# LambdaLabsML/distributed-training-guide

Measured on AMD Instinct MI355X. Metric: tokens/sec/GPU for Llama-style causal LM at 1/2/4/8 MI355X; peak HBM per GPU, higher is better.
Workload: dtype bf16; 1 GPU; model=llama-3-8b, global_batch=24, seq_len=1024, parallelism=single

## Files before the change

distributed_training_guide_amd/_hip/attention_bwd.hip:

```cpp
#include "attention_common.h"
#include "launchers.h"

template <int D>
__global__ void __launch_bounds__(256) attn_delta_kernel(
    const short* __restrict__ dout, const short* __restrict__ o,
    float* __restrict__ delta, int B, int S, int Hq) {
  const int grp = threadIdx.x >> 4;
  const int gl = threadIdx.x & 15;
  int64_t nrows = (int64_t)B * S * Hq;
  for (int64_t row = (int64_t)blockIdx.x * 16 + grp; row < nrows;
       row += (int64_t)gridDim.x * 16) {
    const short* dp = dout + row * D;
    const short* op = o + row * D;
    float s = 0.f;
#pragma unroll
    for (int i = gl * 8; i < D; i += 16 * 8) {
      bf16x8 dv = *reinterpret_cast<const bf16x8*>(dp + i);
      bf16x8 ov = *reinterpret_cast<const bf16x8*>(op + i);
#pragma unroll
      for (int j = 0; j < 8; ++j) s += bf2f(dv[j]) * bf2f(ov[j]);
    }
#pragma unroll
    for (int off = 1; off < 16; off <<= 1) s += __shfl_xor(s, off, WAVE);
    if (gl == 0) {
      int h = (int)(row % Hq);
      int64_t bs = row / Hq;
      int sp = (int)(bs % S);
      int b = (int)(bs / S);
      delta[((int64_t)b * Hq + h) * S + sp] = s;
    }
  }
}

template <int D, bool DOC>
__global__ void __launch_bounds__(256, 2) attn_dkdv_kernel(
    const short* __restrict__ dout, const short* __restrict__ q,
    const short* __restrict__ k, const short* __restrict__ v,
    const float* __restrict__ lse, const float* __restrict__ delta,
    short* __restrict__ dk, short* __restrict__ dv, int B, int S, int Hq,
    int Hkv, float scale, const int* __restrict__ doc_end) {
  static_assert(D == 64 || D == 128, "head dim must be 64 or 128");
  __shared__ short q_lds[2][64 * D];
  __shared__ short do_lds[2][64 * D];
  __shared__ __attribute__((aligned(16))) float lse_lds[2][64];
  __shared__ __attribute__((aligned(16))) float del_lds[2][64];

  const int nkt = (S + 63) / 64;
  const int group = Hq / Hkv;

  const GroupBlock gb = xcd_remap(blockIdx.x, B * Hkv, nkt);
  const int b = gb.gid / Hkv;
  const int hkv = gb.gid % Hkv;
  const int kt = gb.within;

  const int tid = threadIdx.x;
  const int wid = tid >> 6;
  const int lane = tid & (WAVE - 1);
  const int l15 = lane & 15;
  const int lg = lane >> 4;

  const int kv0 = kt * 64 + wid * 16;
  constexpr int nd16 = D >> 4, nkc = D >> 5;
  const float c2 = scale * LOG2E;
  const int64_t strideS_q = (int64_t)Hq * D;
  const int64_t strideS_kv = (int64_t)Hkv * D;
  const short* kb = k + ((int64_t)b * S * Hkv + hkv) * D;
  const short* vb = v + ((int64_t)b * S * Hkv + hkv) * D;

  bf16x8 kf[nkc], vf[nkc];
  {
    int key = kv0 + l15;
    int keyc = key < S ? key : S - 1;
    const short* kp = kb + (int64_t)keyc * strideS_kv + lg * 8;
    const short* vp = vb + (int64_t)keyc * strideS_kv + lg * 8;
#pragma unroll
    for (int c = 0; c < nkc; ++c) {
      kf[c] = *reinterpret_cast<const bf16x8*>(kp + c * 32);
      vf[c] = *reinterpret_cast<const bf16x8*>(vp + c * 32);
    }
  }

  f32x4 dkacc[nd16], dvacc[nd16];
#pragma unroll
  for (int i = 0; i < nd16; ++i) {
    dkacc[i] = {0.f, 0.f, 0.f, 0.f};
    dvacc[i] = {0.f, 0.f, 0.f, 0.f};
  }

  const int qstart = kt * 64;
  int dend = S, dend_min = S, qcap = S;
  if (DOC) {
    const int* deb = doc_end + (int64_t)b * S;
    dend = deb[min(kv0 + l15, S - 1)];
    dend_min = deb[min(kv0, S - 1)];
    qcap = min(max(deb[min(qstart + 63, S - 1)], qstart + 1), S);
  }
  const int nqt = (qcap - qstart + 63) / 64;
  const int niter = group * nqt;

  auto stage_qdo = [&](int it, int buf) {
    const int64_t hoff = ((int64_t)b * S * Hq + hkv * group + it / nqt) * D;
    stage_tile_pair<D>(q + hoff, dout + hoff, strideS_q,
                       qstart + (it % nqt) * 64, S, q_lds[buf], do_lds[buf],
                       wid, lane);
  };
  auto stage_lse = [&](int it, int buf) {
    const int hh = hkv * group + it / nqt;
    const int qt = qstart + (it % nqt) * 64;
    if (tid < 64) {
      const float* lseb = lse + ((int64_t)b * Hq + hh) * S;
      int rr = qt + tid < S ? qt + tid : S - 1;
      lse_lds[buf][tid] = lseb[rr] * LOG2E;
    } else if (tid < 128) {
      const float* delb = delta + ((int64_t)b * Hq + hh) * S;
      int rr = qt + tid - 64 < S ? qt + tid - 64 : S - 1;
      del_lds[buf][tid - 64] = delb[rr] * scale;
    }
  };

  stage_qdo(0, 0);
  stage_lse(0, 0);
  __syncthreads();

  for (int it = 0; it < niter; ++it) {
    const int buf = it & 1;
    if (it + 1 < niter) {
      stage_qdo(it + 1, buf ^ 1);
      stage_lse(it + 1, buf ^ 1);
    }

    const int qt = qstart + (it % nqt) * 64;
    const short* ql = q_lds[buf];
    const short* dol = do_lds[buf];

    const int key = kv0 + l15;
    const bool diag = (qt < kt * 64 + 64) || (qt + 63 >= S) ||
                      (DOC && qt + 63 >= dend_min);
    u32x4 pk_p[2], pk_ds[2];
    __builtin_amdgcn_s_setprio(1);
#pragma unroll
    for (int mth = 0; mth < 2; ++mth) {
      const int qra = perm16(2 * mth, l15), qrb = perm16(2 * mth + 1, l15);
      f32x4 sa0 = {0.f, 0.f, 0.f, 0.f}, da0 = {0.f, 0.f, 0.f, 0.f};
      f32x4 sa1 = {0.f, 0.f, 0.f, 0.f}, da1 = {0.f, 0.f, 0.f, 0.f};
#pragma unroll
      for (int c = 0; c < nkc; ++c) {
        bf16x8 qa0 = *reinterpret_cast<const bf16x8*>(
            ql + st_idx(qra, c * 32 + lg * 8));
        bf16x8 qa1 = *reinterpret_cast<const bf16x8*>(
            ql + st_idx(qrb, c * 32 + lg * 8));
        bf16x8 do0 = *reinterpret_cast<const bf16x8*>(
            dol + st_idx(qra, c * 32 + lg * 8));
        bf16x8 do1 = *reinterpret_cast<const bf16x8*>(
            dol + st_idx(qrb, c * 32 + lg * 8));
        sa0 = mfma16(qa0, kf[c], sa0);
        sa1 = mfma16(qa1, kf[c], sa1);
        da0 = mfma16(do0, vf[c], da0);
        da1 = mfma16(do1, vf[c], da1);
      }
#pragma unroll
      for (int half = 0; half < 2; ++half) {
        const int mt = 2 * mth + half;
        const f32x4 sa = half ? sa1 : sa0;
        const f32x4 da = half ? da1 : da0;
        const int qoff = cpos16(mt, lg);
        const f32x4 lse4 =
            *reinterpret_cast<const f32x4*>(&lse_lds[buf][qoff]);
        const f32x4 del4 =
            *reinterpret_cast<const f32x4*>(&del_lds[buf][qoff]);
        float e[4], p[4], ds[4];
#pragma unroll
        for (int r = 0; r < 4; ++r)
          e[r] = __builtin_fmaf(sa[r], c2, -lse4[r]);
        if (diag) {
#pragma unroll
          for (int r = 0; r < 4; ++r) {
            const int qrow = qt + qoff + r;
            if (key > qrow || qrow >= S || key >= S || (DOC && qrow >= dend))
              e[r] = -INFINITY;
          }
        }
#pragma unroll
        for (int r = 0; r < 4; ++r) {
          p[r] = __builtin_amdgcn_exp2f(e[r]);
          ds[r] = p[r] * __builtin_fmaf(da[r], scale, -del4[r]);
        }
        const int kc = mt >> 1, rp = (mt & 1) * 2;
        pk_p[kc][rp + 0] = cvt_pk_bf16(p[0], p[1]);
        pk_p[kc][rp + 1] = cvt_pk_bf16(p[2], p[3]);
        pk_ds[kc][rp + 0] = cvt_pk_bf16(ds[0], ds[1]);
        pk_ds[kc][rp + 1] = cvt_pk_bf16(ds[2], ds[3]);
      }
    }

#pragma unroll
    for (int dt = 0; dt < nd16; ++dt) {
#pragma unroll
      for (int kc = 0; kc < 2; ++kc) {
        bf16x8 dofr = tr16_frag_st(dol, kc * 32 + lg * 8, dt * 16, l15);
        bf16x8 qfr = tr16_frag_st(ql, kc * 32 + lg * 8, dt * 16, l15);
        dvacc[dt] = mfma16(__builtin_bit_cast(bf16x8, pk_p[kc]), dofr,
                           dvacc[dt]);
        dkacc[dt] = mfma16(__builtin_bit_cast(bf16x8, pk_ds[kc]), qfr,
                           dkacc[dt]);
      }
    }
    __builtin_amdgcn_s_setprio(0);
    __syncthreads();
  }

#pragma unroll
  for (int r = 0; r < 4; ++r) {
    int keyw = kv0 + lg * 4 + r;
    if (keyw >= S) continue;
    short* dkp = dk + ((int64_t)b * S * Hkv + (int64_t)keyw * Hkv + hkv) * D;
    short* dvp = dv + ((int64_t)b * S * Hkv + (int64_t)keyw * Hkv + hkv) * D;
#pragma unroll
    for (int dt = 0; dt < nd16; ++dt) {
      dkp[dt * 16 + l15] = f2bf(dkacc[dt][r]);
      dvp[dt * 16 + l15] = f2bf(dvacc[dt][r]);
    }
  }
}

template <int D, bool DOC>
__global__ void __launch_bounds__(256, 2) attn_dq_kernel(
    const short* __restrict__ dout, const short* __restrict__ q,
    const short* __restrict__ k, const short* __restrict__ v,
    const float* __restrict__ lse, const float* __restrict__ delta,
    short* __restrict__ dq, int B, int S, int Hq, int Hkv, float scale,
    const int* __restrict__ doc_start) {
  static_assert(D == 64 || D == 128, "head dim must be 64 or 128");
  __shared__ short k_lds[2][KVBLK * D];
  __shared__ short v_lds[2][KVBLK * D];

  const int ntq = (S + QBLK - 1) / QBLK;
  const int gqa = Hq / Hkv;
  const int bpg = gqa * ntq;

  const GroupBlock gb = xcd_remap(blockIdx.x, B * Hkv, bpg);
  const int b = gb.gid / Hkv;
  const int hkv = gb.gid % Hkv;
  const int h = hkv * gqa + gb.within / ntq;
  const int qtile = gb.within % ntq;

  const int tid = threadIdx.x;
  const int wid = tid >> 6;
  const int lane = tid & (WAVE - 1);
  const int l15 = lane & 15;
  const int lg = lane >> 4;

  const int q0 = qtile * QBLK;
  const int rowb[2] = {qgroup_row(q0, wid, 0), qgroup_row(q0, wid, 1)};
  constexpr int nd16 = D >> 4, nkc = D >> 5;
  const float c2 = scale * LOG2E;
  const int64_t strideS_q = (int64_t)Hq * D;
  const int64_t strideS_kv = (int64_t)Hkv * D;
  const short* qb = q + ((int64_t)b * S * Hq + h) * D;
  const short* dob = dout + ((int64_t)b * S * Hq + h) * D;
  const short* kb = k + ((int64_t)b * S * Hkv + hkv) * D;
  const short* vb = v + ((int64_t)b * S * Hkv + hkv) * D;
  const float* lseb = lse + ((int64_t)b * Hq + h) * S;
  const float* delb = delta + ((int64_t)b * Hq + h) * S;

  bf16x8 qf[2][nkc], dof[2][nkc];
  float lse_r[2], del_r[2];
#pragma unroll
  for (int nq = 0; nq < 2; ++nq) {
    int qrow = rowb[nq] + l15;
    int qrc = qrow < S ? qrow : S - 1;
    const short* qp = qb + (int64_t)qrc * strideS_q + lg * 8;
    const short* dop = dob + (int64_t)qrc * strideS_q + lg * 8;
#pragma unroll
    for (int c = 0; c < nkc; ++c) {
      qf[nq][c] = *reinterpret_cast<const bf16x8*>(qp + c * 32);
      dof[nq][c] = *reinterpret_cast<const bf16x8*>(dop + c * 32);
    }
    lse_r[nq] = lseb[qrc] * LOG2E;
    del_r[nq] = delb[qrc] * scale;
  }

  f32x4 dqacc[nd16][2];
#pragma unroll
  for (int dt = 0; dt < nd16; ++dt)
#pragma unroll
    for (int nq = 0; nq < 2; ++nq) dqacc[dt][nq] = {0.f, 0.f, 0.f, 0.f};

  const int kv_end = min(S, q0 + QBLK);
  const int ntiles = (kv_end + KVBLK - 1) / KVBLK;
  int dstart[2], dsmax[2];
  const int t0 =
      doc_window<DOC>(doc_start, b, S, q0, wid, l15, dstart, dsmax);

  auto stage_kv = [&](int t, int buf) {
    stage_tile_pair<D>(kb, vb, strideS_kv, t * KVBLK, S, k_lds[buf],
                       v_lds[buf], wid, lane);
  };
  stage_kv(t0, 0);
  __syncthreads();

  for (int t = t0; t < ntiles; ++t) {
    const int kv0 = t * KVBLK;
    const int buf = tile_buf(t, t0);
    if (t + 1 < ntiles) stage_kv(t + 1, buf ^ 1);

    {
      const bool smask = (kv_end < kv0 + KVBLK);
      u32x4 pk_ds[2][2];
      const short* kl = k_lds[buf];
      const short* vl = v_lds[buf];
      __builtin_amdgcn_s_setprio(1);
#pragma unroll
      for (int mt = 0; mt < 4; ++mt) {
        const int kr = perm16(mt, l15);
        f32x4 s0 = {0.f, 0.f, 0.f, 0.f}, s1 = {0.f, 0.f, 0.f, 0.f};
        f32x4 d0 = {0.f, 0.f, 0.f, 0.f}, d1 = {0.f, 0.f, 0.f, 0.f};
#pragma unroll
        for (int c = 0; c < nkc; ++c) {
          bf16x8 ka = *reinterpret_cast<const bf16x8*>(
              kl + st_idx(kr, c * 32 + lg * 8));
          bf16x8 va = *reinterpret_cast<const bf16x8*>(
              vl + st_idx(kr, c * 32 + lg * 8));
          s0 = mfma16(ka, qf[0][c], s0);
          d0 = mfma16(va, dof[0][c], d0);
          s1 = mfma16(ka, qf[1][c], s1);
          d1 = mfma16(va, dof[1][c], d1);
        }
        const int koff = cpos16(mt, lg);
        const int kc = mt >> 1, rp = (mt & 1) * 2;
#pragma unroll
        for (int nq = 0; nq < 2; ++nq) {
          const int qrow = rowb[nq] + l15;
          const bool diag = (kv0 + KVBLK - 1 > rowb[nq]) || smask ||
                            (DOC && dsmax[nq] > kv0);
          const f32x4 sv = nq ? s1 : s0;
          const f32x4 dv = nq ? d1 : d0;
          float e[4], ds[4];
#pragma unroll
          for (int r = 0; r < 4; ++r)
            e[r] = __builtin_fmaf(sv[r], c2, -lse_r[nq]);
          if (diag) {
#pragma unroll
            for (int r = 0; r < 4; ++r) {
              const int keyr = kv0 + koff + r;
              if (keyr > qrow || keyr >= S || qrow >= S ||
                  (DOC && keyr < dstart[nq]))
                e[r] = -INFINITY;
            }
          }
#pragma unroll
          for (int r = 0; r < 4; ++r)
            ds[r] = __builtin_amdgcn_exp2f(e[r]) *
                    __builtin_fmaf(dv[r], scale, -del_r[nq]);
          pk_ds[nq][kc][rp + 0] = cvt_pk_bf16(ds[0], ds[1]);
          pk_ds[nq][kc][rp + 1] = cvt_pk_bf16(ds[2], ds[3]);
        }
      }

#pragma unroll
      for (int dt = 0; dt < nd16; ++dt) {
#pragma unroll
        for (int kc = 0; kc < 2; ++kc) {
          bf16x8 kfr = tr16_frag_st(kl, kc * 32 + lg * 8, dt * 16, l15);
          dqacc[dt][0] = mfma16(__builtin_bit_cast(bf16x8, pk_ds[0][kc]),
                                kfr, dqacc[dt][0]);
          dqacc[dt][1] = mfma16(__builtin_bit_cast(bf16x8, pk_ds[1][kc]),
                                kfr, dqacc[dt][1]);
        }
      }
      __builtin_amdgcn_s_setprio(0);
    }
    __syncthreads();
  }

#pragma unroll
  for (int nq = 0; nq < 2; ++nq) {
#pragma unroll
    for (int r = 0; r < 4; ++r) {
      int qrow = rowb[nq] + lg * 4 + r;
      if (qrow >= S) continue;
      short* dqp = dq + ((int64_t)b * S * Hq + (int64_t)qrow * Hq + h) * D;
#pragma unroll
      for (int dt = 0; dt < nd16; ++dt) {
        dqp[dt * 16 + l15] = f2bf(dqacc[dt][nq][r]);
      }
    }
  }
}

namespace {
template <int D, bool DOC>
void bwd_launch(const short* dout, const short* q, const short* k,
                const short* v, const short* o, const float* lse,
                float* delta, short* dq, short* dk, short* dv,
                const int* doc_start, const int* doc_end, int B, int S,
                int Hq, int Hkv, float scale, hipStream_t stream) {
  int64_t nrows = (int64_t)B * S * Hq;
  int64_t dwant = (nrows + 15) / 16;
  int dgrid = (int)(dwant < 2048 ? (dwant < 1 ? 1 : dwant) : 2048);
  hipLaunchKernelGGL(attn_delta_kernel<D>, dim3(dgrid), dim3(256), 0, stream,
                     dout, o, delta, B, S, Hq);
  int nkt = (S + 63) / 64;
  hipLaunchKernelGGL((attn_dkdv_kernel<D, DOC>),
                     dim3((uint32_t)((int64_t)B * Hkv * nkt)), dim3(256), 0,
                     stream, dout, q, k, v, lse, delta, dk, dv, B, S, Hq, Hkv,
                     scale, doc_end);
  int ntq = (S + QBLK - 1) / QBLK;
  hipLaunchKernelGGL((attn_dq_kernel<D, DOC>),
                     dim3((uint32_t)((int64_t)B * Hq * ntq)), dim3(256), 0,
                     stream, dout, q, k, v, lse, delta, dq, B, S, Hq, Hkv,
                     scale, doc_start);
}
}

extern "C" void attn_bwd_launch(const void* dout, const void* q, const void* k,
                                const void* v, const void* o, const float* lse,
                                float* delta, void* dq, void* dk, void* dv,
                                const int* doc_start, const int* doc_end,
                                int B, int S, int Hq, int Hkv, int D,
                                float scale, hipStream_t stream) {
  const bool doc = doc_start != nullptr;
  auto fn = doc ? (D == 64 ? bwd_launch<64, true> : bwd_launch<128, true>)
                : (D == 64 ? bwd_launch<64, false> : bwd_launch<128, false>);
  fn((const short*)dout, (const short*)q, (const short*)k, (const short*)v,
     (const short*)o, lse, delta, (short*)dq, (short*)dk, (short*)dv,
     doc_start, doc_end, B, S, Hq, Hkv, scale, stream);
}
```

distributed_training_guide_amd/_hip/attention_common.h:

```cpp
#pragma once
#include "common.h"

using bf16x8 = s16x8;

constexpr int QBLK = 128;
constexpr int KVBLK = 64;
#define LOG2E 1.4426950408889634f

__device__ __forceinline__ f32x4 mfma16(bf16x8 a, bf16x8 b, f32x4 c) {
  return __builtin_amdgcn_mfma_f32_16x16x32_bf16(a, b, c, 0, 0, 0);
}

template <int D>
__device__ __forceinline__ void stage_tile_pair(
    const short* ga, const short* gb, int64_t stride, int row0, int S,
    short* la, short* lb, int wid, int lane) {
  constexpr int ncw = D >> 5;
#pragma unroll
  for (int i = 0; i < ncw; ++i) {
    const int ch = wid * ncw + i;
    int row = row0 + (ch & 1) * 32 + (lane >> 1);
    if (row >= S) row = S - 1;
    const int64_t goff =
        (int64_t)row * stride + (ch >> 1) * 16 + (lane & 1) * 8;
    __builtin_amdgcn_global_load_lds(
        (const __attribute__((address_space(1))) unsigned int*)(ga + goff),
        (LDS_AS unsigned int*)(la + ch * 512), 16, 0, 0);
    __builtin_amdgcn_global_load_lds(
        (const __attribute__((address_space(1))) unsigned int*)(gb + goff),
        (LDS_AS unsigned int*)(lb + ch * 512), 16, 0, 0);
  }
}

struct GroupBlock {
  int gid;
  int within;
};
__device__ __forceinline__ GroupBlock xcd_remap(int bid, int ngroups,
                                                int bpg) {
  if ((ngroups & 7) == 0)
    return {(bid >> 3) / bpg * 8 + (bid & 7), (bid >> 3) % bpg};
  return {bid / bpg, bid % bpg};
}

__device__ __forceinline__ int qgroup_row(int q0, int wid, int nq) {
  return q0 + nq * 64 + wid * 16;
}

template <bool DOC>
__device__ __forceinline__ int doc_window(const int* doc_start, int b, int S,
                                          int q0, int wid, int l15,
                                          int (&dstart)[2], int (&dsmax)[2]) {
  dstart[0] = dstart[1] = dsmax[0] = dsmax[1] = 0;
  if (!DOC) return 0;
  const int* dsb = doc_start + (int64_t)b * S;
#pragma unroll
  for (int nq = 0; nq < 2; ++nq) {
    dstart[nq] = dsb[min(qgroup_row(q0, wid, nq) + l15, S - 1)];
    dsmax[nq] = dsb[min(qgroup_row(q0, wid, nq) + 15, S - 1)];
  }
  return min(max(dsb[q0], 0), q0) / KVBLK;
}

__device__ __forceinline__ int tile_buf(int t, int t0) { return (t - t0) & 1; }
```

distributed_training_guide_amd/_hip/attention_fwd.hip:

```cpp
#include "attention_common.h"
#include "launchers.h"

template <int D, bool DOC>
__global__ void __launch_bounds__(256, 2) attn_fwd_kernel(
    const short* __restrict__ q, const short* __restrict__ k,
    const short* __restrict__ v, short* __restrict__ o,
    float* __restrict__ lse_out, int B, int S, int Hq, int Hkv, float scale,
    const int* __restrict__ doc_start) {
  static_assert(D == 64 || D == 128, "head dim must be 64 or 128");
  __shared__ short k_lds[2][KVBLK * D];
  __shared__ short v_lds[2][KVBLK * D];

  const int ntq = (S + QBLK - 1) / QBLK;
  const int gqa = Hq / Hkv;
  const int bpg = gqa * ntq;

  const GroupBlock gb = xcd_remap(blockIdx.x, B * Hkv, bpg);
  const int b = gb.gid / Hkv;
  const int hkv = gb.gid % Hkv;
  const int h = hkv * gqa + gb.within / ntq;
  const int qtile = gb.within % ntq;

  const int tid = threadIdx.x;
  const int wid = tid >> 6;
  const int lane = tid & (WAVE - 1);
  const int l15 = lane & 15;
  const int lg = lane >> 4;

  const int q0 = qtile * QBLK;
  const int rowb[2] = {qgroup_row(q0, wid, 0), qgroup_row(q0, wid, 1)};
  constexpr int nd16 = D >> 4;
  constexpr int nkc = D >> 5;
  const int64_t strideS_q = (int64_t)Hq * D;
  const int64_t strideS_kv = (int64_t)Hkv * D;
  const short* qb = q + ((int64_t)b * S * Hq + h) * D;
  const short* kb = k + ((int64_t)b * S * Hkv + hkv) * D;
  const short* vb = v + ((int64_t)b * S * Hkv + hkv) * D;

  bf16x8 qf[2][nkc];
#pragma unroll
  for (int nq = 0; nq < 2; ++nq) {
    int qrow = rowb[nq] + l15;
    if (qrow >= S) qrow = S - 1;
    const short* qp = qb + (int64_t)qrow * strideS_q + lg * 8;
#pragma unroll
    for (int kc = 0; kc < nkc; ++kc)
      qf[nq][kc] = *reinterpret_cast<const bf16x8*>(qp + kc * 32);
  }

  int kperm[4], ckey[4];
#pragma unroll
  for (int mt = 0; mt < 4; ++mt) {
    kperm[mt] = perm16(mt, l15);
    ckey[mt] = cpos16(mt, lg);
  }

  f32x4 oacc[nd16][2];
#pragma unroll
  for (int dt = 0; dt < nd16; ++dt)
#pragma unroll
    for (int nq = 0; nq < 2; ++nq) oacc[dt][nq] = {0.f, 0.f, 0.f, 0.f};
  float mrow[2] = {-INFINITY, -INFINITY};
  float mcrow[2] = {-INFINITY, -INFINITY};
  float lrow[2] = {0.f, 0.f};

  const int kv_end = min(S, q0 + QBLK);
  const int ntiles = (kv_end + KVBLK - 1) / KVBLK;
  const float c = scale * LOG2E;
  int dstart[2], dsmax[2];
  const int t0 =
      doc_window<DOC>(doc_start, b, S, q0, wid, l15, dstart, dsmax);

  auto stage_kv = [&](int t, int buf) {
    stage_tile_pair<D>(kb, vb, strideS_kv, t * KVBLK, S, k_lds[buf],
                       v_lds[buf], wid, lane);
  };
  stage_kv(t0, 0);
  __syncthreads();

  for (int t = t0; t < ntiles; ++t) {
    const int kv0 = t * KVBLK;
    const int buf = tile_buf(t, t0);
    if (t + 1 < ntiles) stage_kv(t + 1, buf ^ 1);


    const short* kl = k_lds[buf];
    f32x4 sfrag[4][2];
    __builtin_amdgcn_s_setprio(1);
#pragma unroll
    for (int mth = 0; mth < 2; ++mth) {
      const int kra = kperm[2 * mth], krb = kperm[2 * mth + 1];
      f32x4 a0 = {0.f, 0.f, 0.f, 0.f}, a1 = {0.f, 0.f, 0.f, 0.f};
      f32x4 b0 = {0.f, 0.f, 0.f, 0.f}, b1 = {0.f, 0.f, 0.f, 0.f};
#pragma unroll
      for (int kc = 0; kc < nkc; ++kc) {
        bf16x8 kfa = *reinterpret_cast<const bf16x8*>(
            kl + st_idx(kra, kc * 32 + lg * 8));
        bf16x8 kfb = *reinterpret_cast<const bf16x8*>(
            kl + st_idx(krb, kc * 32 + lg * 8));
        a0 = mfma16(kfa, qf[0][kc], a0);
        b0 = mfma16(kfb, qf[0][kc], b0);
        a1 = mfma16(kfa, qf[1][kc], a1);
        b1 = mfma16(kfb, qf[1][kc], b1);
      }
      sfrag[2 * mth][0] = a0;
      sfrag[2 * mth][1] = a1;
      sfrag[2 * mth + 1][0] = b0;
      sfrag[2 * mth + 1][1] = b1;
    }
    __builtin_amdgcn_s_setprio(0);

    u32x4 pk[2][2];
    float alpha[2];
#pragma unroll
    for (int nq = 0; nq < 2; ++nq) {
      const int qrow = rowb[nq] + l15;
      const bool need_mask = (kv0 + KVBLK - 1) > rowb[nq] ||
                             kv_end < kv0 + KVBLK ||
                             (DOC && dsmax[nq] > kv0);
      if (need_mask) {
#pragma unroll
        for (int mt = 0; mt < 4; ++mt)
#pragma unroll
          for (int r = 0; r < 4; ++r) {
            int key = kv0 + ckey[mt] + r;
            if (key > qrow || key >= S || (DOC && key < dstart[nq]))
              sfrag[mt][nq][r] = -INFINITY;
          }
      }
      float tmax = -INFINITY;
#pragma unroll
      for (int mt = 0; mt < 4; ++mt) {
        f32x4 s = sfrag[mt][nq];
        tmax = fmaxf(tmax, fmaxf(fmaxf(s[0], s[1]), fmaxf(s[2], s[3])));
      }
      tmax = fmaxf(tmax, __shfl_xor(tmax, 16, WAVE));
      tmax = fmaxf(tmax, __shfl_xor(tmax, 32, WAVE));
      const float mnew = fmaxf(mrow[nq], tmax);
      const float mcn = mnew * c;
      const float mc = (mnew == -INFINITY) ? 0.0f : mcn;
      alpha[nq] = __builtin_amdgcn_exp2f(mcrow[nq] - mc);
      mrow[nq] = mnew;
      mcrow[nq] = mcn;
      float psum = 0.f;
#pragma unroll
      for (int mt = 0; mt < 4; ++mt) {
        f32x4 s = sfrag[mt][nq];
        f32x4 p;
#pragma unroll
        for (int r = 0; r < 4; ++r) {
          p[r] = __builtin_amdgcn_exp2f(__builtin_fmaf(s[r], c, -mc));
          psum += p[r];
        }
        pk[nq][mt >> 1][(mt & 1) * 2 + 0] = cvt_pk_bf16(p[0], p[1]);
        pk[nq][mt >> 1][(mt & 1) * 2 + 1] = cvt_pk_bf16(p[2], p[3]);
      }
      psum += __shfl_xor(psum, 16, WAVE);
      psum += __shfl_xor(psum, 32, WAVE);
      lrow[nq] = lrow[nq] * alpha[nq] + psum;
    }

    const short* vt = v_lds[buf];
    __builtin_amdgcn_s_setprio(1);
#pragma unroll
    for (int dt = 0; dt < nd16; ++dt) {
      bf16x8 va[2];
#pragma unroll
      for (int kc = 0; kc < 2; ++kc)
        va[kc] = tr16_frag_st(vt, kc * 32 + lg * 8, dt * 16, l15);
#pragma unroll
      for (int nq = 0; nq < 2; ++nq) {
        f32x4 acc = oacc[dt][nq];
#pragma unroll
        for (int r = 0; r < 4; ++r) acc[r] *= alpha[nq];
        acc = mfma16(va[0], __builtin_bit_cast(bf16x8, pk[nq][0]), acc);
        acc = mfma16(va[1], __builtin_bit_cast(bf16x8, pk[nq][1]), acc);
        oacc[dt][nq] = acc;
      }
    }
    __builtin_amdgcn_s_setprio(0);
    __syncthreads();
  }

#pragma unroll
  for (int nq = 0; nq < 2; ++nq) {
    const int qrow = rowb[nq] + l15;
    if (qrow >= S) continue;
    const float invl = (lrow[nq] > 0.f) ? 1.0f / lrow[nq] : 0.0f;
    short* op = o + ((int64_t)b * S * Hq + (int64_t)qrow * Hq + h) * D;
#pragma unroll
    for (int dt = 0; dt < nd16; ++dt) {
      s16x4 outv;
#pragma unroll
      for (int r = 0; r < 4; ++r) outv[r] = f2bf(oacc[dt][nq][r] * invl);
      *reinterpret_cast<s16x4*>(op + dt * 16 + lg * 4) = outv;
    }
    if (lg == 0)
      lse_out[((int64_t)b * Hq + h) * S + qrow] =
          mrow[nq] * scale + __logf(fmaxf(lrow[nq], 1e-30f));
  }
}

extern "C" void attn_fwd_launch(const void* q, const void* k, const void* v,
                                void* o, float* lse, const int* doc_start,
                                int B, int S, int Hq, int Hkv, int D,
                                float scale, hipStream_t stream) {
  int ntiles = (S + QBLK - 1) / QBLK;
  int64_t grid = (int64_t)B * Hq * ntiles;
  auto kern = doc_start
                  ? (D == 64 ? attn_fwd_kernel<64, true>
                             : attn_fwd_kernel<128, true>)
                  : (D == 64 ? attn_fwd_kernel<64, false>
                             : attn_fwd_kernel<128, false>);
  hipLaunchKernelGGL(kern, dim3((uint32_t)grid), dim3(256), 0, stream,
                     (const short*)q, (const short*)k, (const short*)v,
                     (short*)o, lse, B, S, Hq, Hkv, scale, doc_start);
}
```

Baseline: 24620 tokens/s.

## Use inline-asm LDS DMA, reverse q-tile order, stage dQ/O stores through LDS

Replaces the builtin global_load_lds with inline asm that sets m0 explicitly and adds explicit vmcnt waits and register pins to control when loads complete. Adds register prefetch of LSE/delta in the dK/dV kernel, and reverses q-tile scheduling in the forward and dQ kernels so the longest causal tiles start first. The forward O and backward dQ epilogues now write through LDS and store coalesced 16-byte rows instead of scattered 2- or 8-byte stores. These changes aim to cut load-sync overhead, tail imbalance and uncoalesced global writes, at the cost of fragile inline asm and extra waits.

```diff
diff --git a/distributed_training_guide_amd/_hip/attention_bwd.hip b/distributed_training_guide_amd/_hip/attention_bwd.hip
--- a/distributed_training_guide_amd/_hip/attention_bwd.hip
+++ b/distributed_training_guide_amd/_hip/attention_bwd.hip
@@ -104,30 +104,37 @@
                        qstart + (it % nqt) * 64, S, q_lds[buf], do_lds[buf],
                        wid, lane);
   };
-  auto stage_lse = [&](int it, int buf) {
+  auto load_ld = [&](int it) -> float {
     const int hh = hkv * group + it / nqt;
     const int qt = qstart + (it % nqt) * 64;
-    if (tid < 64) {
-      const float* lseb = lse + ((int64_t)b * Hq + hh) * S;
-      int rr = qt + tid < S ? qt + tid : S - 1;
-      lse_lds[buf][tid] = lseb[rr] * LOG2E;
-    } else if (tid < 128) {
-      const float* delb = delta + ((int64_t)b * Hq + hh) * S;
-      int rr = qt + tid - 64 < S ? qt + tid - 64 : S - 1;
-      del_lds[buf][tid - 64] = delb[rr] * scale;
-    }
+    const float* src = (tid & 64 ? delta : lse) + ((int64_t)b * Hq + hh) * S;
+    return src[min(qt + (tid & 63), S - 1)];
   };
+  auto put_ld = [&](int buf, float raw) {
+    if (tid < 64)
+      lse_lds[buf][tid] = raw * LOG2E;
+    else if (tid < 128)
+      del_lds[buf][tid - 64] = raw * scale;
+  };
 
   stage_qdo(0, 0);
-  stage_lse(0, 0);
+  put_ld(0, load_ld(0));
+#pragma unroll
+  for (int c = 0; c < nkc; ++c) {
+    pin_loaded(kf[c]);
+    pin_loaded(vf[c]);
+  }
+  if (DOC) {
+    pin_loaded(dend);
+    pin_loaded(dend_min);
+  }
+  dma_wait();
   __syncthreads();
 
   for (int it = 0; it < niter; ++it) {
     const int buf = it & 1;
-    if (it + 1 < niter) {
-      stage_qdo(it + 1, buf ^ 1);
-      stage_lse(it + 1, buf ^ 1);
-    }
+    float ld_next = load_ld(min(it + 1, niter - 1));
+    if (it + 1 < niter) stage_qdo(it + 1, buf ^ 1);
 
     const int qt = qstart + (it % nqt) * 64;
     const short* ql = q_lds[buf];
@@ -206,6 +213,9 @@
       }
     }
     __builtin_amdgcn_s_setprio(0);
+    dma_wait();
+    pin_loaded(ld_next);
+    put_ld(buf ^ 1, ld_next);
     __syncthreads();
   }
 
@@ -242,7 +252,7 @@
   const int b = gb.gid / Hkv;
   const int hkv = gb.gid % Hkv;
   const int h = hkv * gqa + gb.within / ntq;
-  const int qtile = gb.within % ntq;
+  const int qtile = ntq - 1 - gb.within % ntq;
 
   const int tid = threadIdx.x;
   const int wid = tid >> 6;
@@ -297,6 +307,21 @@
                        v_lds[buf], wid, lane);
   };
   stage_kv(t0, 0);
+#pragma unroll
+  for (int nq = 0; nq < 2; ++nq) {
+#pragma unroll
+    for (int c = 0; c < nkc; ++c) {
+      pin_loaded(qf[nq][c]);
+      pin_loaded(dof[nq][c]);
+    }
+    pin_loaded(lse_r[nq]);
+    pin_loaded(del_r[nq]);
+    if (DOC) {
+      pin_loaded(dstart[nq]);
+      pin_loaded(dsmax[nq]);
+    }
+  }
+  dma_wait();
   __syncthreads();
 
   for (int t = t0; t < ntiles; ++t) {
@@ -370,22 +395,27 @@
       }
       __builtin_amdgcn_s_setprio(0);
     }
+    dma_wait();
     __syncthreads();
   }
 
-#pragma unroll
-  for (int nq = 0; nq < 2; ++nq) {
-#pragma unroll
-    for (int r = 0; r < 4; ++r) {
-      int qrow = rowb[nq] + lg * 4 + r;
-      if (qrow >= S) continue;
-      short* dqp = dq + ((int64_t)b * S * Hq + (int64_t)qrow * Hq + h) * D;
-#pragma unroll
-      for (int dt = 0; dt < nd16; ++dt) {
-        dqp[dt * 16 + l15] = f2bf(dqacc[dt][nq][r]);
-      }
-    }
-  }
+  static_assert(2 * 32 * OROW<D> <= 2 * KVBLK * D, "fits one tile array");
+  short* wl = (wid < 2 ? &k_lds[0][0] : &v_lds[0][0]) +
+              (wid & 1) * 32 * OROW<D>;
+#pragma unroll
+  for (int nq = 0; nq < 2; ++nq)
+#pragma unroll
+    for (int r = 0; r < 4; ++r)
+#pragma unroll
+      for (int dt = 0; dt < nd16; ++dt)
+        wl[(nq * 16 + lg * 4 + r) * OROW<D> + dt * 16 + l15] =
+            f2bf(dqacc[dt][nq][r]);
+  store_rows<D, 32>(wl, lane, [&](int r) -> short* {
+    const int qrow = rowb[r >> 4] + (r & 15);
+    return qrow < S
+               ? dq + ((int64_t)b * S * Hq + (int64_t)qrow * Hq + h) * D
+               : nullptr;
+  });
 }
 
 namespace {
diff --git a/distributed_training_guide_amd/_hip/attention_common.h b/distributed_training_guide_amd/_hip/attention_common.h
--- a/distributed_training_guide_amd/_hip/attention_common.h
+++ b/distributed_training_guide_amd/_hip/attention_common.h
@@ -11,11 +11,36 @@
   return __builtin_amdgcn_mfma_f32_16x16x32_bf16(a, b, c, 0, 0, 0);
 }
 
+__device__ __forceinline__ void glds16(const short* gsrc, unsigned lds_dst) {
+  unsigned keep;
+  asm volatile(
+      "s_mov_b32 %0, m0\n\t"
+      "s_mov_b32 m0, %2\n\t"
+      "s_nop 0\n\t"
+      "global_load_lds_dwordx4 %1, off\n\t"
+      "s_mov_b32 m0, %0"
+      : "=&s"(keep)
+      : "v"(gsrc), "s"(lds_dst)
+      : "memory");
+}
+
+__device__ __forceinline__ void dma_wait() {
+  asm volatile("s_waitcnt vmcnt(0)" ::: "memory");
+}
+
+template <typename T>
+__device__ __forceinline__ void pin_loaded(T& x) {
+  asm volatile("" : "+v"(x));
+}
+
 template <int D>
 __device__ __forceinline__ void stage_tile_pair(
     const short* ga, const short* gb, int64_t stride, int row0, int S,
     short* la, short* lb, int wid, int lane) {
   constexpr int ncw = D >> 5;
+  const int wu = __builtin_amdgcn_readfirstlane(wid);
+  const unsigned la0 = (unsigned)(uintptr_t)(LDS_AS short*)la;
+  const unsigned lb0 = (unsigned)(uintptr_t)(LDS_AS short*)lb;
 #pragma unroll
   for (int i = 0; i < ncw; ++i) {
     const int ch = wid * ncw + i;
@@ -23,12 +48,29 @@
     if (row >= S) row = S - 1;
     const int64_t goff =
         (int64_t)row * stride + (ch >> 1) * 16 + (lane & 1) * 8;
-    __builtin_amdgcn_global_load_lds(
-        (const __attribute__((address_space(1))) unsigned int*)(ga + goff),
-        (LDS_AS unsigned int*)(la + ch * 512), 16, 0, 0);
-    __builtin_amdgcn_global_load_lds(
-        (const __attribute__((address_space(1))) unsigned int*)(gb + goff),
-        (LDS_AS unsigned int*)(lb + ch * 512), 16, 0, 0);
+    const unsigned loff = (unsigned)(wu * ncw + i) * 1024u;
+    glds16(ga + goff, la0 + loff);
+    glds16(gb + goff, lb0 + loff);
+  }
+}
+
+template <int D>
+constexpr int OROW = D + 8;
+
+template <int D, int NROWS, typename RowPtr>
+__device__ __forceinline__ void store_rows(const short* wl, int lane,
+                                           RowPtr grow) {
+  constexpr int lpr = D / 8;
+  constexpr int rpi = 64 / lpr;
+  static_assert(NROWS % rpi == 0, "whole wave instructions only");
+  asm volatile("s_waitcnt lgkmcnt(0)" ::: "memory");
+#pragma unroll
+  for (int i = 0; i < NROWS / rpi; ++i) {
+    const int r = i * rpi + lane / lpr;
+    const int c = (lane % lpr) * 8;
+    const bf16x8 val = *reinterpret_cast<const bf16x8*>(wl + r * OROW<D> + c);
+    short* gp = grow(r);
+    if (gp) *reinterpret_cast<bf16x8*>(gp + c) = val;
   }
 }
 
diff --git a/distributed_training_guide_amd/_hip/attention_fwd.hip b/distributed_training_guide_amd/_hip/attention_fwd.hip
--- a/distributed_training_guide_amd/_hip/attention_fwd.hip
+++ b/distributed_training_guide_amd/_hip/attention_fwd.hip
@@ -19,7 +19,7 @@
   const int b = gb.gid / Hkv;
   const int hkv = gb.gid % Hkv;
   const int h = hkv * gqa + gb.within / ntq;
-  const int qtile = gb.within % ntq;
+  const int qtile = ntq - 1 - gb.within % ntq;
 
   const int tid = threadIdx.x;
   const int wid = tid >> 6;
@@ -76,6 +76,16 @@
                        v_lds[buf], wid, lane);
   };
   stage_kv(t0, 0);
+#pragma unroll
+  for (int nq = 0; nq < 2; ++nq) {
+#pragma unroll
+    for (int kc = 0; kc < nkc; ++kc) pin_loaded(qf[nq][kc]);
+    if (DOC) {
+      pin_loaded(dstart[nq]);
+      pin_loaded(dsmax[nq]);
+    }
+  }
+  dma_wait();
   __syncthreads();
 
   for (int t = t0; t < ntiles; ++t) {
@@ -179,26 +189,35 @@
       }
     }
     __builtin_amdgcn_s_setprio(0);
+    dma_wait();
     __syncthreads();
   }
 
+  static_assert(2 * 32 * OROW<D> <= 2 * KVBLK * D, "fits one tile array");
+  short* wl = (wid < 2 ? &k_lds[0][0] : &v_lds[0][0]) +
+              (wid & 1) * 32 * OROW<D>;
 #pragma unroll
   for (int nq = 0; nq < 2; ++nq) {
-    const int qrow = rowb[nq] + l15;
-    if (qrow >= S) continue;
     const float invl = (lrow[nq] > 0.f) ? 1.0f / lrow[nq] : 0.0f;
-    short* op = o + ((int64_t)b * S * Hq + (int64_t)qrow * Hq + h) * D;
 #pragma unroll
     for (int dt = 0; dt < nd16; ++dt) {
       s16x4 outv;
 #pragma unroll
       for (int r = 0; r < 4; ++r) outv[r] = f2bf(oacc[dt][nq][r] * invl);
-      *reinterpret_cast<s16x4*>(op + dt * 16 + lg * 4) = outv;
-    }
-    if (lg == 0)
+      *reinterpret_cast<s16x4*>(wl + (nq * 16 + l15) * OROW<D> + dt * 16 +
+                                lg * 4) = outv;
+    }
+    const int qrow = rowb[nq] + l15;
+    if (lg == 0 && qrow < S)
       lse_out[((int64_t)b * Hq + h) * S + qrow] =
           mrow[nq] * scale + __logf(fmaxf(lrow[nq], 1e-30f));
   }
+  store_rows<D, 32>(wl, lane, [&](int r) -> short* {
+    const int qrow = rowb[r >> 4] + (r & 15);
+    return qrow < S
+               ? o + ((int64_t)b * S * Hq + (int64_t)qrow * Hq + h) * D
+               : nullptr;
+  });
 }
 
 extern "C" void attn_fwd_launch(const void* q, const void* k, const void* v,
```

New measurement: 24710 tokens/s (median of 6 runs). Within noise of the previous version (+0.4%).
